# thesteve0/llm-fine-tune-distributed

Measured on AMD Instinct MI355X. Metric: samples/sec SmolLM3-3B full SFT bf16 (DDP), higher is better.
Workload: dtype bf16

## Files before the change

csrc/attention.hip:

```cpp
#include "common.h"

#include <cstring>

namespace sftamd {

namespace attn {

constexpr int D = 128;
constexpr int ROWB = D * 2;
constexpr float LOG2E = 1.4426950408889634f;
constexpr float LN2 = 0.6931471805599453f;

__device__ __forceinline__ int swz(int row, int ch) {
  return ch ^ (((row & 3) << 2) | ((0x78 >> (2 * ((row >> 2) & 3))) & 3));
}
__device__ __forceinline__ int img_off(int row, int ch) { return row * ROWB + 16 * swz(row, ch); }

__device__ __forceinline__ f32x4 mfma(const bf16x8& a, const bf16x8& b, const f32x4& c) {
  return __builtin_amdgcn_mfma_f32_16x16x32_bf16(a, b, c, 0, 0, 0);
}

template <int R, int NT>
__device__ __forceinline__ void stage(char* lds, const u16* __restrict__ g, long ld, int nvalid, int tid) {
#pragma unroll
  for (int it = 0; it < (R * 16) / NT; ++it) {
    const int idx = tid + it * NT;
    const int r = idx >> 4, ch = idx & 15;
    uint4 v = make_uint4(0, 0, 0, 0);
    if (r < nvalid) v = *(const uint4*)(g + (long)r * ld + ch * 8);
    *(uint4*)(lds + img_off(r, ch)) = v;
  }
}


__device__ __forceinline__ bf16x8 pack_acc(const f32x4& t0, const f32x4& t1) {
  typedef __attribute__((ext_vector_type(4))) unsigned w4;
  return __builtin_bit_cast(bf16x8, w4{pk2bf(t0[0], t0[1]), pk2bf(t0[2], t0[3]), pk2bf(t1[0], t1[1]), pk2bf(t1[2], t1[3])});
}

__device__ __forceinline__ bf16x8 load_frag_global(const u16* p, bool ok) {
  if (!ok) return bf16x8{};
  return __builtin_bit_cast(bf16x8, *(const uint4*)p);
}

__device__ __forceinline__ void store4(u16* p, const f32x4& v, float s) {
  uint2 w;
  w.x = pk2bf(v[0] * s, v[1] * s);
  w.y = pk2bf(v[2] * s, v[3] * s);
  *(uint2*)p = w;
}


__global__ __launch_bounds__(256) void delta_kernel(const u16* __restrict__ dout, const u16* __restrict__ out,
                                                    float* __restrict__ delta, int total, int nq) {
  const long rowid = blockIdx.x * 16L + (threadIdx.x >> 4);
  const int sub = threadIdx.x & 15;
  float s = 0.f;
  const bool ok = rowid < (long)total * nq;
  if (ok) {
    const long base = rowid * D + sub * 8;
    float a[8], c[8];
    unpack8(*(const uint4*)(dout + base), a);
    unpack8(*(const uint4*)(out + base), c);
#pragma unroll
    for (int i = 0; i < 8; ++i) s += a[i] * c[i];
  }
#pragma unroll
  for (int o = 8; o > 0; o >>= 1) s += __shfl_xor(s, o, 16);
  if (ok && sub == 0) {
    const long m = rowid / nq;
    const int h = (int)(rowid - m * nq);
    delta[(long)h * total + m] = s;
  }
}

constexpr float THR = 8.f;

struct Offs {
  int row[4];
  int tr[8];
  __device__ __forceinline__ void init(int lane) {
    const int g = lane >> 4, r = lane & 15;
#pragma unroll
    for (int s = 0; s < 4; ++s) row[s] = img_off(r, 4 * s + g);
    const int q = r >> 2, p = r & 3, r0 = 4 * g + q;
#pragma unroll
    for (int dt = 0; dt < 8; ++dt) tr[dt] = img_off(r0, 2 * dt + (p >> 1)) + 8 * (p & 1);
  }
};

__device__ __forceinline__ bf16x8 lds_row(const char* base, int off) { return *(const bf16x8*)(base + off); }

__device__ __forceinline__ bf16x8 lds_tr(const char* base, int off) {
  typedef __attribute__((address_space(3))) s16x4 lds_s4;
  s16x4 lo = __builtin_amdgcn_ds_read_tr16_b64_v4i16((lds_s4*)(base + off));
  s16x4 hi = __builtin_amdgcn_ds_read_tr16_b64_v4i16((lds_s4*)(base + off + 16 * ROWB));
  typedef __attribute__((ext_vector_type(8))) short s16x8;
  s16x8 v = {lo[0], lo[1], lo[2], lo[3], hi[0], hi[1], hi[2], hi[3]};
  return __builtin_bit_cast(bf16x8, v);
}

__device__ __forceinline__ void vm_drain() { __builtin_amdgcn_s_waitcnt(0x0F70); }

typedef float f32x2 __attribute__((ext_vector_type(2)));
__device__ __forceinline__ float max3f(float a, float b, float c) {
  float r;
  asm("v_max3_f32 %0, %1, %2, %3" : "=v"(r) : "v"(a), "v"(b), "v"(c));
  return r;
}

template <int R, int NT>
struct Stage {
  static constexpr int N = (R * 16) / NT;
  uint4 v[N];
  __device__ __forceinline__ void load(const u16* __restrict__ g, long ld, int nvalid, int tid) {
    const int r = tid >> 4, ch = tid & 15;
    const u16* p = g + (long)r * ld + ch * 8;
    if (nvalid >= R) {
#pragma unroll
      for (int it = 0; it < N; ++it) v[it] = *(const uint4*)(p + (long)it * (NT / 16) * ld);
    } else {
#pragma unroll
      for (int it = 0; it < N; ++it)
        v[it] = (r + it * (NT / 16) < nvalid) ? *(const uint4*)(p + (long)it * (NT / 16) * ld) : make_uint4(0, 0, 0, 0);
    }
  }
  __device__ __forceinline__ void store(char* lds, int tid) const {
    const int off = img_off(tid >> 4, tid & 15);
#pragma unroll
    for (int it = 0; it < N; ++it) *(uint4*)(lds + off + it * (NT / 16) * ROWB) = v[it];
  }
};


typedef __amdgpu_buffer_rsrc_t rsrc_t;
__device__ __forceinline__ rsrc_t make_rsrc(const void* p, long bytes) {
  const unsigned long long a = (unsigned long long)p;
  const unsigned lo = __builtin_amdgcn_readfirstlane((unsigned)a), hi = __builtin_amdgcn_readfirstlane((unsigned)(a >> 32));
  const unsigned n = __builtin_amdgcn_readfirstlane((unsigned)(bytes < 0 ? 0 : bytes));
  return __builtin_amdgcn_make_buffer_rsrc((void*)(((unsigned long long)hi << 32) | lo), 0, n, 0x00020000);
}
__device__ __forceinline__ void bdma16(rsrc_t r, char* dst, unsigned voff, unsigned soff) {
  __builtin_amdgcn_raw_ptr_buffer_load_lds(r, (__attribute__((address_space(3))) void*)dst, 16, voff, soff, 0, 0);
}
__device__ __forceinline__ bf16x8 bload16(rsrc_t r, unsigned voff) {
  const auto v = __builtin_amdgcn_raw_buffer_load_b128(r, voff, 0, 0);
  return __builtin_bit_cast(bf16x8, v);
}

typedef __attribute__((ext_vector_type(16))) float f32x16;

__device__ __forceinline__ f32x16 mfma32(const bf16x8& a, const bf16x8& b, const f32x16& c) {
  return __builtin_amdgcn_mfma_f32_32x32x16_bf16(a, b, c, 0, 0, 0);
}

struct Offs32 {
  int k[8];
  int v[8];
  __device__ __forceinline__ void init(int lane) {
    const int c = lane & 31, hi = lane >> 5, a = lane >> 4, q = (lane & 15) >> 2, p = lane & 3;
#pragma unroll
    for (int s = 0; s < 8; ++s) k[s] = img_off(c, 2 * s + hi);
#pragma unroll
    for (int db = 0; db < 4; ++db)
#pragma unroll
      for (int part = 0; part < 2; ++part)
        v[2 * db + part] = img_off(8 * part + 4 * hi + q, 4 * db + 2 * (a & 1) + (p >> 1)) + 8 * (p & 1);
  }
};

__device__ __forceinline__ bf16x8 lds_tr2(const char* base, int lo, int hi) {
  typedef __attribute__((address_space(3))) s16x4 lds_s4;
  s16x4 a = __builtin_amdgcn_ds_read_tr16_b64_v4i16((lds_s4*)(base + lo));
  s16x4 b = __builtin_amdgcn_ds_read_tr16_b64_v4i16((lds_s4*)(base + hi));
  typedef __attribute__((ext_vector_type(8))) short s16x8;
  s16x8 v = {a[0], a[1], a[2], a[3], b[0], b[1], b[2], b[3]};
  return __builtin_bit_cast(bf16x8, v);
}

typedef __attribute__((ext_vector_type(4))) unsigned u32x4;
__device__ __forceinline__ u32x4 pack8w(const f32x16& t, int base) {
  return u32x4{pk2bf(t[base], t[base + 1]), pk2bf(t[base + 2], t[base + 3]), pk2bf(t[base + 4], t[base + 5]),
               pk2bf(t[base + 6], t[base + 7])};
}
__device__ __forceinline__ bf16x8 pack8(const f32x16& t, int base) {
  return __builtin_bit_cast(bf16x8, pack8w(t, base));
}

__device__ __forceinline__ float swap32max(float x) {
  auto a = __builtin_amdgcn_permlane32_swap(__float_as_uint(x), __float_as_uint(x), false, false);
  return fmaxf(__uint_as_float(a[0]), __uint_as_float(a[1]));
}
__device__ __forceinline__ float swap32sum(float x) {
  auto a = __builtin_amdgcn_permlane32_swap(__float_as_uint(x), __float_as_uint(x), false, false);
  return __uint_as_float(a[0]) + __uint_as_float(a[1]);
}

__device__ __forceinline__ void store_t21(u16* row, const f32x16 (&a)[4], float s, bool ok) {
  const int hi = (threadIdx.x >> 5) & 1;
#pragma unroll
  for (int db = 0; db < 4; ++db)
#pragma unroll
    for (int u = 0; u < 2; ++u) {
      const int i0 = 8 * u;
      const unsigned ax = pk2bf(a[db][i0] * s, a[db][i0 + 1] * s);
      const unsigned ay = pk2bf(a[db][i0 + 2] * s, a[db][i0 + 3] * s);
      const unsigned bx = pk2bf(a[db][i0 + 4] * s, a[db][i0 + 5] * s);
      const unsigned by = pk2bf(a[db][i0 + 6] * s, a[db][i0 + 7] * s);
      const auto rx = __builtin_amdgcn_permlane32_swap(ax, bx, false, false);
      const auto ry = __builtin_amdgcn_permlane32_swap(ay, by, false, false);
      if (ok) *(uint4*)(row + 32 * db + 16 * u + 8 * hi) = make_uint4(rx[0], ry[0], rx[1], ry[1]);
    }
}

__device__ __forceinline__ void fwd32_step(const char* __restrict__ cur, char* __restrict__ nxt, bool pre, rsrc_t kv,
                                           unsigned voffk, unsigned voffv, unsigned rowb, int wave, int k0, int lastkey,
                                           bool need_mask, int rel, float sl2, const Offs32& off,
                                           const bf16x8 (&qf)[8], f32x16 (&o)[4], float& m, float& l) {
  constexpr int TB = 64 * ROWB;
  if (pre) {
#pragma unroll
    for (int j = 0; j < 4; ++j) {
      const unsigned so = (unsigned)(k0 + 64 + 16 * j) * rowb;
      bdma16(kv, nxt + (wave + 4 * j) * 1024, voffk, so);
      bdma16(kv, nxt + TB + (wave + 4 * j) * 1024, voffv, so);
    }
  }
  if (k0 > lastkey) return;
  const bool two = k0 + 32 <= lastkey;
  const char* Ks = cur;
  const char* Vs = cur + TB;
  f32x16 s[2];
  s[0] = mfma32(lds_row(Ks, off.k[0]), qf[0], f32x16{});
#pragma unroll
  for (int st = 1; st < 8; ++st) s[0] = mfma32(lds_row(Ks, off.k[st]), qf[st], s[0]);
  if (two) {
    s[1] = mfma32(lds_row(Ks, off.k[0] + 32 * ROWB), qf[0], f32x16{});
#pragma unroll
    for (int st = 1; st < 8; ++st) s[1] = mfma32(lds_row(Ks, off.k[st] + 32 * ROWB), qf[st], s[1]);
  } else {
#pragma unroll
    for (int i = 0; i < 16; ++i) s[1][i] = -INFINITY;
  }
  if (need_mask) {
#pragma unroll
    for (int kb = 0; kb < 2; ++kb)
#pragma unroll
      for (int i = 0; i < 16; ++i)
        s[kb][i] = 32 * kb + (i & 3) + 8 * (i >> 2) > rel ? -INFINITY : s[kb][i];
  }
  float mx = max3f(s[0][0], s[0][1], s[0][2]);
#pragma unroll
  for (int i = 3; i < 15; i += 2) mx = max3f(mx, s[0][i], s[0][i + 1]);
  mx = max3f(mx, s[0][15], s[1][0]);
#pragma unroll
  for (int i = 1; i < 15; i += 2) mx = max3f(mx, s[1][i], s[1][i + 1]);
  mx = fmaxf(mx, s[1][15]);
  const float tmax = swap32max(mx) * sl2;
  if (__any(tmax > m + THR)) {
    const float mnew = fmaxf(m, tmax);
    const float alpha = exp2f(m - mnew);
    l *= alpha;
#pragma unroll
    for (int db = 0; db < 4; ++db) o[db] *= alpha;
    m = mnew;
  }
  float acc0 = 0.f, acc1 = 0.f;
#pragma unroll
  for (int kb = 0; kb < 2; ++kb)
#pragma unroll
    for (int i = 0; i < 16; i += 2) {
      const float p0 = exp2f(__builtin_fmaf(s[kb][i], sl2, -m));
      const float p1 = exp2f(__builtin_fmaf(s[kb][i + 1], sl2, -m));
      s[kb][i] = p0;
      s[kb][i + 1] = p1;
      acc0 += p0;
      acc1 += p1;
    }
  l += acc0 + acc1;
#pragma unroll
  for (int ks = 0; ks < 4; ++ks) {
    if (ks >= 2 && !two) break;
    const bf16x8 pb = pack8(s[ks >> 1], 8 * (ks & 1));
#pragma unroll
    for (int db = 0; db < 4; ++db)
      o[db] = mfma32(lds_tr2(Vs, off.v[2 * db] + 16 * ks * ROWB, off.v[2 * db + 1] + 16 * ks * ROWB), pb, o[db]);
  }
}

template <int HW>
__global__ __launch_bounds__(256, 2) void fwd32_kernel(const u16* __restrict__ qkv, u16* __restrict__ out,
                                                       float* __restrict__ lse, const int* __restrict__ cu, int nq,
                                                       int nkv, int total, float sl2, int causal) {
  constexpr int PB = 4 / HW, TB = 64 * ROWB;
  __shared__ __attribute__((aligned(16))) char smem[4 * TB];
  const int b = blockIdx.y, qb = gridDim.z - 1 - blockIdx.z;
  const int start = cu[b], len = cu[b + 1] - start;
  SFT_DASSERT(start >= 0 && len >= 0 && start + len <= total);
  const int q0 = qb * 32 * PB;
  if (q0 >= len) return;
  const int tid = threadIdx.x, lane = tid & 63, wave = __builtin_amdgcn_readfirstlane(tid >> 6), hi = lane >> 5;
  const int h = blockIdx.x * HW + wave % HW;
  const int kvh = (blockIdx.x * HW) / (nq / nkv);
  const long ld = (long)(nq + 2 * nkv) * D;
  const int wq0 = q0 + 32 * (wave / HW);
  const int qi = wq0 + (lane & 31);
  const bool qok = qi < len;
  const int nkb = (len + 63) / 64;
  const int nkt = causal ? min((min(q0 + 32 * PB, len) - 1) / 64 + 1, nkb) : nkb;
  const int lastkey = causal ? min(wq0 + 31, len - 1) : len - 1;
  const int lim = causal ? min(len - 1, qi) : len - 1;
  Offs32 off;
  off.init(lane);
  const unsigned rowb = (unsigned)ld * 2;
  bf16x8 qf[8];
  {
    const rsrc_t qr = make_rsrc(qkv + (long)start * ld + h * D, (long)(len - 1) * ld * 2 + ROWB);
    const unsigned vo = (unsigned)qi * rowb + 16 * hi;
#pragma unroll
    for (int st = 0; st < 8; ++st) qf[st] = bload16(qr, vo + 32 * st);
  }
  const rsrc_t kv = make_rsrc(qkv + (long)start * ld + (nq + kvh) * D, (long)len * ld * 2 - (long)(nq + kvh) * ROWB);
  const int r0 = 4 * wave + (lane >> 4);
  const unsigned voffk = (unsigned)r0 * rowb + 16 * swz(r0, lane & 15), voffv = voffk + nkv * ROWB;
#pragma unroll
  for (int j = 0; j < 4; ++j) {
    bdma16(kv, smem + (wave + 4 * j) * 1024, voffk, 16 * j * rowb);
    bdma16(kv, smem + TB + (wave + 4 * j) * 1024, voffv, 16 * j * rowb);
  }
  vm_drain();
  f32x16 o[4];
#pragma unroll
  for (int db = 0; db < 4; ++db)
#pragma unroll
    for (int i = 0; i < 16; ++i) o[db][i] = 0.f;
  float m = -1e30f, l = 0.f;
  __syncthreads();
  for (int kt = 0; kt < nkt; ++kt) {
    const int k0 = kt * 64;
    const bool pre = kt + 1 < nkt;
    const bool need_mask = (k0 + 64 > len) || (causal && k0 + 63 > wq0);
    fwd32_step(smem + (kt & 1) * 2 * TB, smem + ((kt + 1) & 1) * 2 * TB, pre, kv, voffk, voffv, rowb, wave, k0,
               lastkey, need_mask, lim - k0 - 4 * hi, sl2, off, qf, o, m, l);
    if (pre) vm_drain();
    __syncthreads();
  }
  l = swap32sum(l);
  const float inv = 1.f / l;
  store_t21(out + (long)(start + qi) * nq * D + h * D, o, inv, qok);
  if (qok && hi == 0) lse[(long)h * total + start + qi] = (m + log2f(l)) * LN2;
}

template <int NW>
__global__ __launch_bounds__(NW * 64) void bwd_dq3_kernel(const u16* __restrict__ qkv, const u16* __restrict__ dout,
                                                          const float* __restrict__ lse,
                                                          const float* __restrict__ delta, const int* __restrict__ cu,
                                                          u16* __restrict__ dqkv, int nq, int nkv, int total,
                                                          float sl2, float scale, int causal) {
  constexpr int NT = NW * 64, BM = NW * 16, TB = 64 * ROWB;
  __shared__ __attribute__((aligned(16))) char smem[2 * TB];
  char* Ks = smem;
  char* Vs = smem + TB;
  const int h = blockIdx.x, b = blockIdx.y, qb = gridDim.z - 1 - blockIdx.z;
  const int start = cu[b], len = cu[b + 1] - start;
  SFT_DASSERT(start >= 0 && len >= 0 && start + len <= total);
  const int q0 = qb * BM;
  if (q0 >= len) return;
  const int kvh = h / (nq / nkv);
  const long ld = (long)(nq + 2 * nkv) * D;
  const long ldo = (long)nq * D;
  const int tid = threadIdx.x, lane = tid & 63, wave = tid >> 6, g = lane >> 4;
  const int wfirst = q0 + wave * 16;
  const int qrow = wfirst + (lane & 15);
  const bool qok = qrow < len;
  const u16* kbase = qkv + (long)start * ld + (nq + kvh) * D;
  const u16* vbase = qkv + (long)start * ld + (nq + nkv + kvh) * D;
  const int nkb = (len + 63) / 64;
  const int nkt = causal ? min((q0 + BM + 63) / 64, nkb) : nkb;
  Offs off;
  off.init(lane);
  {
    Stage<64, NT> tk, tv;
    tk.load(kbase, ld, len, tid);
    tv.load(vbase, ld, len, tid);
    tk.store(Ks, tid);
    tv.store(Vs, tid);
  }
  bf16x8 qf[4], df[4];
  {
    const u16* qp = qkv + (long)(start + qrow) * ld + h * D + 8 * g;
    const u16* dp = dout + (long)(start + qrow) * ldo + h * D + 8 * g;
#pragma unroll
    for (int s = 0; s < 4; ++s) {
      qf[s] = load_frag_global(qp + 32 * s, qok);
      df[s] = load_frag_global(dp + 32 * s, qok);
    }
  }
  const float lse2 = qok ? lse[(long)h * total + start + qrow] * LOG2E : 0.f;
  const float dl = qok ? delta[(long)h * total + start + qrow] : 0.f;
  f32x4 dq[8];
#pragma unroll
  for (int dt = 0; dt < 8; ++dt) dq[dt] = f32x4{0.f, 0.f, 0.f, 0.f};
  __syncthreads();
  for (int kt = 0; kt < nkt; ++kt) {
    const int k0 = kt * 64;
    const bool pre = kt + 1 < nkt;
    Stage<64, NT> tk, tv;
    if (pre) {
      tk.load(kbase + (long)(k0 + 64) * ld, ld, len - k0 - 64, tid);
      tv.load(vbase + (long)(k0 + 64) * ld, ld, len - k0 - 64, tid);
    }
    if (!causal || k0 <= wfirst + 15) {
      f32x4 sc[4], dp[4];
#pragma unroll
      for (int nt = 0; nt < 4; ++nt) {
        sc[nt] = f32x4{0.f, 0.f, 0.f, 0.f};
        dp[nt] = f32x4{0.f, 0.f, 0.f, 0.f};
#pragma unroll
        for (int s = 0; s < 4; ++s) {
          sc[nt] = mfma(lds_row(Ks, off.row[s] + nt * 16 * ROWB), qf[s], sc[nt]);
          dp[nt] = mfma(lds_row(Vs, off.row[s] + nt * 16 * ROWB), df[s], dp[nt]);
        }
      }
      const bool need_mask = (k0 + 64 > len) || (causal && k0 + 63 > wfirst) || (q0 + BM > len);
#pragma unroll
      for (int nt = 0; nt < 4; ++nt)
#pragma unroll
        for (int i = 0; i < 4; ++i) {
          float p = exp2f(fmaf(sc[nt][i], sl2, -lse2));
          if (need_mask) {
            const int key = k0 + 16 * nt + 4 * g + i;
            if (key >= len || (causal && key > qrow) || !qok) p = 0.f;
          }
          dp[nt][i] = p * (dp[nt][i] - dl);
        }
#pragma unroll
      for (int ks = 0; ks < 2; ++ks) {
        const bf16x8 db = pack_acc(dp[2 * ks], dp[2 * ks + 1]);
#pragma unroll
        for (int dt = 0; dt < 8; ++dt) dq[dt] = mfma(lds_tr(Ks, off.tr[dt] + ks * 32 * ROWB), db, dq[dt]);
      }
    }
    if (pre) {
      __syncthreads();
      tk.store(Ks, tid);
      tv.store(Vs, tid);
    }
    __syncthreads();
  }
  if (qok) {
    u16* qp = dqkv + (long)(start + qrow) * ld + h * D + 4 * g;
#pragma unroll
    for (int dt = 0; dt < 8; ++dt) store4(qp + 16 * dt, dq[dt], scale);
  }
}

__device__ __forceinline__ void rope_bwd32(f32x16 (&a)[4], const float* cs, const float* sn, float s) {
  const int hi = (threadIdx.x >> 5) & 1;
#pragma unroll
  for (int d4 = 0; d4 < 2; ++d4)
#pragma unroll
    for (int m = 0; m < 4; ++m) {
      const int d = 32 * d4 + 8 * m + 4 * hi;
      const float4 c4 = *(const float4*)(cs + d), s4 = *(const float4*)(sn + d);
      const float c[4] = {c4.x, c4.y, c4.z, c4.w}, n[4] = {s4.x, s4.y, s4.z, s4.w};
#pragma unroll
      for (int t = 0; t < 4; ++t) {
        const int i = 4 * m + t;
        const float x = a[d4][i] * s, y = a[d4 + 2][i] * s;
        a[d4][i] = x * c[t] + y * n[t];
        a[d4 + 2][i] = y * c[t] - x * n[t];
      }
    }
}

__device__ __forceinline__ void dq32_step(const char* __restrict__ cur, char* __restrict__ nxt, bool pre, bool active,
                                          rsrc_t kr, rsrc_t sr, unsigned voffk, unsigned voffs, unsigned rowb,
                                          unsigned rows, int k0n, int wave, const Offs32& off, int sofs,
                                          f32x16 (&dq)[4]) {
  constexpr int TB = 64 * ROWB, SB = 64 * 64;
  if (pre) {
#pragma unroll
    for (int j = 0; j < 4; ++j) {
      bdma16(kr, nxt + (wave + 4 * j) * 1024, voffk, (unsigned)(k0n + 16 * j) * rowb);
      bdma16(sr, nxt + TB + wave * SB + j * 1024, voffs, (unsigned)(k0n + 16 * j) * rows);
    }
  }
  if (!active) return;
  const char* Ks = cur;
  const char* Ss = cur + TB + wave * SB;
#pragma unroll
  for (int ks = 0; ks < 4; ++ks) {
    const bf16x8 sb = lds_tr2(Ss, sofs + ks * 16 * 64, sofs + ks * 16 * 64 + 8 * 64);
#pragma unroll
    for (int d4 = 0; d4 < 4; ++d4)
      dq[d4] = mfma32(lds_tr2(Ks, off.v[2 * d4] + ks * 16 * ROWB, off.v[2 * d4 + 1] + ks * 16 * ROWB), sb, dq[d4]);
  }
}

template <int HW>
__global__ __launch_bounds__(256, 2) void bwd_dq32_kernel(const u16* __restrict__ qkv, const u16* __restrict__ dst,
                                                          const int* __restrict__ cu, u16* __restrict__ dqkv, int nq,
                                                          int nkv, int lp, float scale, int causal,
                                                          const float* __restrict__ rcos,
                                                          const float* __restrict__ rsin) {
  constexpr int PB = 4 / HW, TB = 64 * ROWB, SB = 64 * 64, STG = TB + 4 * SB;
  __shared__ __attribute__((aligned(16))) char smem[2 * STG];
  const int b = blockIdx.y, qb = gridDim.z - 1 - blockIdx.z;
  const int start = cu[b], len = cu[b + 1] - start;
  const int q0 = qb * 32 * PB;
  if (q0 >= len) return;
  const int tid = threadIdx.x, lane = tid & 63, wave = __builtin_amdgcn_readfirstlane(tid >> 6), hi = lane >> 5;
  const int h = blockIdx.x * HW + wave % HW;
  const int kvh = (blockIdx.x * HW) / (nq / nkv);
  const long ld = (long)(nq + 2 * nkv) * D;
  const int wq0 = q0 + 32 * (wave / HW);
  const int qi = wq0 + (lane & 31);
  SFT_DASSERT(wq0 + 32 <= lp);
  const int lastq = min(wq0 + 31, len - 1);
  const u16* kbase = qkv + (long)start * ld + (nq + kvh) * D;
  const u16* sbase = dst + (long)(b * nq + h) * lp * lp + wq0;
  const int nkb = (len + 63) / 64;
  const int nkt = causal ? min((min(q0 + 32 * PB, len) - 1) / 64 + 1, nkb) : nkb;
  Offs32 off;
  off.init(lane);
  const int sofs = (4 * hi + ((lane & 15) >> 2)) * 64 + 32 * ((lane >> 4) & 1) + 8 * (lane & 3);
  const int r0 = 4 * wave + (lane >> 4);
  const unsigned rowb = (unsigned)ld * 2, rows = (unsigned)lp * 2;
  const rsrc_t kr = make_rsrc(kbase, (long)(len - 1) * ld * 2 + ROWB);
  const rsrc_t sr = make_rsrc(sbase, (long)(len - 1) * lp * 2 + 64);
  const unsigned voffk = (unsigned)r0 * rowb + 16 * swz(r0, lane & 15);
  const unsigned voffs = (unsigned)(lane >> 2) * rows + 16 * (lane & 3);
  f32x16 dq[4];
#pragma unroll
  for (int d4 = 0; d4 < 4; ++d4)
#pragma unroll
    for (int i = 0; i < 16; ++i) dq[d4][i] = 0.f;
  dq32_step(smem + STG, smem, true, false, kr, sr, voffk, voffs, rowb, rows, 0, wave, off, sofs, dq);
  vm_drain();
  __syncthreads();
  for (int kt = 0; kt < nkt; ++kt) {
    const int k0 = kt * 64;
    const bool pre = kt + 1 < nkt;
    dq32_step(smem + (kt & 1) * STG, smem + ((kt + 1) & 1) * STG, pre, !causal || k0 <= lastq, kr, sr, voffk, voffs,
              rowb, rows, k0 + 64, wave, off, sofs, dq);
    if (pre) vm_drain();
    __syncthreads();
  }
  const bool qok = qi < len;
  float s = scale;
  if (rcos != nullptr && qok) {
    const long tr = (long)(start + qi) * (D / 2);
    rope_bwd32(dq, rcos + tr, rsin + tr, scale);
    s = 1.f;
  }
  store_t21(dqkv + (long)(start + qi) * ld + h * D, dq, s, qok);
}

__device__ __forceinline__ void dkdv32_step(const char* __restrict__ cur, char* __restrict__ nxt, bool pre,
                                            rsrc_t qr, rsrc_t orr, unsigned vq0, unsigned vq1, unsigned vo0,
                                            unsigned vo1, unsigned qso, unsigned oso, unsigned rowb, unsigned rowo,
                                            int wv, const float* lsrc, const float* dsrc, int gl, int q0, int len,
                                            int causal, int kw0, int key, float sl2, u16* drow,
                                            const Offs32& off, const bf16x8 (&kf)[8], const char* Vk,
                                            f32x16 (&dk)[4], f32x16 (&dv)[4]) {
  constexpr int TB = 64 * ROWB;
  float pl = 0.f, pd = 0.f;
  if (pre) {
#pragma unroll
    for (int j = 0; j < 8; ++j) {
      bdma16(qr, nxt + (wv + 2 * j) * 1024, (j & 1) ? vq1 : vq0, qso + 16 * (j >> 1) * rowb);
      bdma16(orr, nxt + TB + (wv + 2 * j) * 1024, (j & 1) ? vo1 : vo0, oso + 16 * (j >> 1) * rowo);
    }
    if (gl < 64 && lsrc != nullptr) {
      pl = lsrc[gl];
      pd = dsrc[gl];
    }
  }
  const char* Qs = cur;
  const char* Os = cur + TB;
  const float* Ls = (const float*)(cur + 2 * TB);
  const float* Dl = Ls + 64;
  const int hi = (threadIdx.x >> 5) & 1;
  const bool wds = __builtin_amdgcn_readfirstlane((int)(drow != nullptr));
#pragma unroll 1
  for (int qb = 0; qb < 2; ++qb) {
    f32x16 s, dp;
#pragma unroll
    for (int i = 0; i < 16; ++i) s[i] = dp[i] = 0.f;
#pragma unroll
    for (int st = 0; st < 8; ++st) {
      s = mfma32(lds_row(Qs, off.k[st] + qb * 32 * ROWB), kf[st], s);
      dp = mfma32(lds_row(Os, off.k[st] + qb * 32 * ROWB), lds_row(Vk, off.k[st]), dp);
    }
    const int qbase = q0 + 32 * qb + 4 * hi;
    const int lo = (causal ? key : 0) - qbase, hq = len - 1 - qbase;
    const bool need_mask = (q0 + 32 * qb + 31 >= len) || (causal && kw0 + 31 > q0 + 32 * qb);
#pragma unroll
    for (int m = 0; m < 4; ++m) {
      const float4 L4 = *(const float4*)(Ls + 32 * qb + 8 * m + 4 * hi);
      const float4 D4 = *(const float4*)(Dl + 32 * qb + 8 * m + 4 * hi);
      const float L[4] = {L4.x, L4.y, L4.z, L4.w}, Dd[4] = {D4.x, D4.y, D4.z, D4.w};
#pragma unroll
      for (int t = 0; t < 4; ++t) {
        const int i = 4 * m + t;
        const float p = exp2f(__builtin_fmaf(s[i], sl2, -L[t]));
        dp[i] = p * (dp[i] - Dd[t]);
        s[i] = p;
      }
    }
    if (need_mask) {
      int vlo = lo, vhi = hq;
      asm volatile("" : "+v"(vlo), "+v"(vhi));
#pragma unroll
      for (int i = 0; i < 16; ++i) {
        const int o = 8 * (i >> 2) + (i & 3);
        if (o < vlo || o > vhi) s[i] = dp[i] = 0.f;
      }
    }
#pragma unroll
    for (int sub = 0; sub < 2; ++sub) {
      const u32x4 dw = pack8w(dp, 8 * sub);
      if (wds) {
        const auto rx = __builtin_amdgcn_permlane32_swap(dw[0], dw[2], false, false);
        const auto ry = __builtin_amdgcn_permlane32_swap(dw[1], dw[3], false, false);
        *(uint4*)(drow + 32 * qb + 16 * sub + 8 * hi) = make_uint4(rx[0], ry[0], rx[1], ry[1]);
      }
      const bf16x8 pb = pack8(s, 8 * sub), db = __builtin_bit_cast(bf16x8, dw);
      const int ko = (2 * qb + sub) * 16 * ROWB;
#pragma unroll
      for (int d4 = 0; d4 < 4; ++d4) {
        dv[d4] = mfma32(lds_tr2(Os, off.v[2 * d4] + ko, off.v[2 * d4 + 1] + ko), pb, dv[d4]);
        dk[d4] = mfma32(lds_tr2(Qs, off.v[2 * d4] + ko, off.v[2 * d4 + 1] + ko), db, dk[d4]);
      }
    }
  }
  if (pre && gl < 64) {
    float* Ln = (float*)(nxt + 2 * TB);
    asm volatile("" : "+v"(pl));
    Ln[gl] = pl * LOG2E;
    Ln[64 + gl] = pd;
  }
}

template <int G>
__global__ __launch_bounds__(128 * G, 1) void bwd_dkdv32_kernel(
    const u16* __restrict__ qkv, const u16* __restrict__ dout, const float* __restrict__ lse,
    const float* __restrict__ delta, const int* __restrict__ cu, u16* __restrict__ dqkv, int nq, int nkv, int total,
    float sl2, float scale, int causal, u16* __restrict__ dst, int lp, const float* __restrict__ rcos,
    const float* __restrict__ rsin) {
  constexpr int TB = 64 * ROWB, GB = 2 * TB + 2 * 64 * 4;
  __shared__ __attribute__((aligned(16))) char smem[G * 2 * GB + TB];
  const int tid = threadIdx.x, lane = tid & 63, w = __builtin_amdgcn_readfirstlane(tid >> 6), grp = w >> 1, kh = w & 1;
  const int gl = tid & 127;
  const int hi = lane >> 5;
  char* base = smem + grp * 2 * GB;
  const int kvh = blockIdx.x, b = blockIdx.y, kb = blockIdx.z;
  const int start = cu[b], len = cu[b + 1] - start;
  SFT_DASSERT(start >= 0 && len >= 0 && start + len <= total);
  const int k0 = kb * 64;
  if (k0 >= len) return;
  const int rep = nq / nkv, hpg = rep / G;
  const long ld = (long)(nq + 2 * nkv) * D;
  const long ldo = (long)nq * D;
  const int kw0 = k0 + 32 * kh, key = kw0 + (lane & 31);
  const bool kok = key < len;
  const int qt0 = causal ? kb : 0, nqt = (len + 63) / 64, nt = nqt - qt0, niter = hpg * nt;
  Offs32 off;
  off.init(lane);
  int h = kvh * rep + grp * hpg, qt = qt0;
  const int qr0 = 4 * kh + (lane >> 4);
  const unsigned rowb = (unsigned)ld * 2, rowo = (unsigned)ldo * 2;
  const rsrc_t qr = make_rsrc(qkv + (long)start * ld, (long)(len - 1) * ld * 2 + (long)nq * ROWB);
  const rsrc_t orr = make_rsrc(dout + (long)start * ldo, (long)len * ldo * 2);
  const unsigned sw0 = 16 * swz(qr0, lane & 15), sw1 = 16 * swz(qr0 + 8, lane & 15);
  const unsigned vq0 = (unsigned)qr0 * rowb + sw0, vq1 = (unsigned)(qr0 + 8) * rowb + sw1;
  const unsigned vo0 = (unsigned)qr0 * rowo + sw0, vo1 = (unsigned)(qr0 + 8) * rowo + sw1;
  {
    const int q0 = qt0 * 64, qv = len - q0;
#pragma unroll
    for (int j = 0; j < 8; ++j) {
      bdma16(qr, base + (kh + 2 * j) * 1024, (j & 1) ? vq1 : vq0, (unsigned)(q0 + 16 * (j >> 1)) * rowb + h * ROWB);
      bdma16(orr, base + TB + (kh + 2 * j) * 1024, (j & 1) ? vo1 : vo0, (unsigned)(q0 + 16 * (j >> 1)) * rowo + h * ROWB);
    }
    if (gl < 64) {
      float* Ls = (float*)(base + 2 * TB);
      Ls[gl] = gl < qv ? lse[(long)h * total + start + q0 + gl] * LOG2E : 0.f;
      Ls[64 + gl] = gl < qv ? delta[(long)h * total + start + q0 + gl] : 0.f;
    }
  }
  bf16x8 kf[8];
  char* Vk = smem + G * 2 * GB + kh * 32 * ROWB;
  {
    const rsrc_t kr = make_rsrc(qkv + (long)start * ld + (nq + kvh) * D, (long)(len - 1) * ld * 2 + (long)(nkv + 1) * ROWB);
    const unsigned vo = (unsigned)key * rowb + 16 * hi;
#pragma unroll
    for (int st = 0; st < 8; ++st) kf[st] = bload16(kr, vo + 32 * st);
    const int vr = 4 * w + (lane >> 4);
    const unsigned vv0 = (unsigned)(k0 + vr) * rowb + nkv * ROWB + 16 * swz(vr, lane & 15);
    const unsigned vv1 = (unsigned)(k0 + vr) * rowb + nkv * ROWB + 16 * swz(vr + 8, lane & 15);
#pragma unroll
    for (int j = 0; j < 8 / G; ++j)
      bdma16(kr, smem + G * 2 * GB + (w + 2 * G * j) * 1024, (G == 1 && (j & 1)) ? vv1 : vv0,
             (unsigned)(8 * G * j) * rowb);
  }
  vm_drain();
  f32x16 dk[4], dv[4];
#pragma unroll
  for (int d4 = 0; d4 < 4; ++d4)
#pragma unroll
    for (int i = 0; i < 16; ++i) dk[d4][i] = dv[d4][i] = 0.f;
  __syncthreads();
  for (int it = 0; it < niter; ++it) {
    const int q0 = qt * 64;
    const bool pre = it + 1 < niter;
    int hn = h, qtn = qt + 1;
    if (qtn == nqt) {
      qtn = qt0;
      ++hn;
    }
    const int qn = qtn * 64;
    const long lo = (long)hn * total + start + qn;
    const bool lok = pre && qn + gl < len;
    u16* drow = dst != nullptr ? dst + ((long)(b * nq + h) * lp + key) * lp + q0 : nullptr;
    dkdv32_step(base + (it & 1) * GB, base + ((it + 1) & 1) * GB, pre, qr, orr, vq0, vq1, vo0, vo1,
                (unsigned)qn * rowb + hn * ROWB, (unsigned)qn * rowo + hn * ROWB, rowb, rowo, kh,
                lok ? lse + lo : nullptr, delta + lo, gl, q0, len, causal, kw0, key, sl2, drow, off, kf, Vk, dk,
                dv);
    if (pre) vm_drain();
    __syncthreads();
    h = hn;
    qt = qtn;
  }
  if constexpr (G == 2) {
    float4* xk = (float4*)smem;
    float4* xv = xk + 2 * 16 * 64;
    if (grp == 1) {
#pragma unroll
      for (int d4 = 0; d4 < 4; ++d4)
#pragma unroll
        for (int v = 0; v < 4; ++v) {
          const int ix = (kh * 16 + 4 * d4 + v) * 64 + lane;
          xk[ix] = make_float4(dk[d4][4 * v], dk[d4][4 * v + 1], dk[d4][4 * v + 2], dk[d4][4 * v + 3]);
          xv[ix] = make_float4(dv[d4][4 * v], dv[d4][4 * v + 1], dv[d4][4 * v + 2], dv[d4][4 * v + 3]);
        }
    }
    __syncthreads();
    if (grp == 1) return;
#pragma unroll
    for (int d4 = 0; d4 < 4; ++d4)
#pragma unroll
      for (int v = 0; v < 4; ++v) {
        const int ix = (kh * 16 + 4 * d4 + v) * 64 + lane;
        const float4 a = xk[ix], c = xv[ix];
        dk[d4][4 * v] += a.x;
        dk[d4][4 * v + 1] += a.y;
        dk[d4][4 * v + 2] += a.z;
        dk[d4][4 * v + 3] += a.w;
        dv[d4][4 * v] += c.x;
        dv[d4][4 * v + 1] += c.y;
        dv[d4][4 * v + 2] += c.z;
        dv[d4][4 * v + 3] += c.w;
      }
  }
  float ks = scale;
  if (rcos != nullptr && kok) {
    const long tr = (long)(start + key) * (D / 2);
    rope_bwd32(dk, rcos + tr, rsin + tr, scale);
    ks = 1.f;
  }
  store_t21(dqkv + (long)(start + key) * ld + (nq + kvh) * D, dk, ks, kok);
  store_t21(dqkv + (long)(start + key) * ld + (nq + nkv + kvh) * D, dv, 1.f, kok);
}

static void launch_dkdv(const u16* qkv, const u16* dout, const float* lse, const float* delta, const int* cu,
                        u16* dqkv, int nq, int nkv, int total, int nseq, int max_seqlen, float sl2, float scale,
                        int causal, u16* dst, int lp, hipStream_t st, const float* rcos = nullptr,
                        const float* rsin = nullptr) {
  dim3 grid(nkv, nseq, (max_seqlen + 63) / 64);
  if ((nq / nkv) % 2 == 0)
    bwd_dkdv32_kernel<2><<<grid, 256, 0, st>>>(qkv, dout, lse, delta, cu, dqkv, nq, nkv, total, sl2, scale, causal,
                                               dst, lp, rcos, rsin);
  else
    bwd_dkdv32_kernel<1><<<grid, 128, 0, st>>>(qkv, dout, lse, delta, cu, dqkv, nq, nkv, total, sl2, scale, causal,
                                               dst, lp, rcos, rsin);
}

}

static void check_attn_args(const at::Tensor& qkv, const at::Tensor& cu, int64_t nq, int64_t nkv, int64_t hd) {
  SFT_CHECK_CUDA(qkv);
  SFT_CHECK_BF16(qkv);
  SFT_CHECK_CONTIG(qkv);
  SFT_CHECK(hd == attn::D, "flash attention kernel is built for head_dim 128, got ", hd);
  SFT_CHECK(nq % nkv == 0, "nq must be a multiple of nkv");
  SFT_CHECK(qkv.dim() == 2 && qkv.size(1) == (nq + 2 * nkv) * hd, "qkv must be [M, (nq+2nkv)*hd]");
  SFT_CHECK(cu.scalar_type() == at::kInt && cu.is_cuda() && cu.dim() == 1 && cu.numel() >= 2, "cu_seqlens int32");
}

static long attn_ds_budget() {
  const char* e = std::getenv("SFTAMD_ATTN_DS_MB");
  return (e && e[0] ? atol(e) : 2048L) * 1024L * 1024L;
}

std::tuple<at::Tensor, at::Tensor> flash_fwd(const at::Tensor& qkv, const at::Tensor& cu, int64_t max_seqlen,
                                             int64_t nq, int64_t nkv, int64_t hd, double scale, bool causal) {
  check_attn_args(qkv, cu, nq, nkv, hd);
  const int total = qkv.size(0);
  const int nseq = cu.numel() - 1;
  auto out = at::empty({total, nq * hd}, qkv.options());
  auto lse = at::empty({nq, total}, qkv.options().dtype(at::kFloat));
  if (total == 0 || max_seqlen == 0) return {out, lse};
  const float sl2 = (float)scale * attn::LOG2E;
  auto cu_c = cu.contiguous();
  const u16* q = (const u16*)qkv.data_ptr();
  u16* o = (u16*)out.data_ptr();
  float* lp = lse.data_ptr<float>();
  const int* cp = cu_c.data_ptr<int>();
  const int ca = causal ? 1 : 0;
  SFT_TRACE("attn.fwd32");
  const int rep = nq / nkv, hw = rep % 4 == 0 ? 4 : rep % 2 == 0 ? 2 : 1, span = 32 * (4 / hw);
  dim3 g(nq / hw, nseq, (max_seqlen + span - 1) / span);
  if (hw == 4) attn::fwd32_kernel<4><<<g, 256, 0, cur_stream()>>>(q, o, lp, cp, nq, nkv, total, sl2, ca);
  else if (hw == 2) attn::fwd32_kernel<2><<<g, 256, 0, cur_stream()>>>(q, o, lp, cp, nq, nkv, total, sl2, ca);
  else attn::fwd32_kernel<1><<<g, 256, 0, cur_stream()>>>(q, o, lp, cp, nq, nkv, total, sl2, ca);
  SFT_LAUNCH_CHECK();
  return {out, lse};
}

static at::Tensor flash_bwd_impl(const at::Tensor& dout, const at::Tensor& qkv, const at::Tensor& out,
                                 const at::Tensor& lse, const at::Tensor& cu, int64_t max_seqlen, int64_t nq,
                                 int64_t nkv, int64_t hd, double scale, bool causal, const float* rcos,
                                 const float* rsin, bool& rope_done, const c10::optional<at::Tensor>& delta_in) {
  rope_done = false;
  check_attn_args(qkv, cu, nq, nkv, hd);
  SFT_CHECK_CONTIG(dout);
  SFT_CHECK_CONTIG(out);
  SFT_CHECK(dout.sizes() == out.sizes() && out.size(1) == nq * hd, "dout/out shape");
  const int total = qkv.size(0);
  const int nseq = cu.numel() - 1;
  auto dqkv = at::empty_like(qkv);
  if (total == 0 || max_seqlen == 0) return dqkv;
  at::Tensor delta;
  if (delta_in.has_value() && delta_in->defined()) {
    delta = *delta_in;
    SFT_CHECK(delta.scalar_type() == at::kFloat && delta.is_contiguous() && delta.dim() == 2 && delta.size(0) == nq &&
                  delta.size(1) == total && delta.device() == qkv.device(),
              "flash_bwd: delta must be contiguous fp32 [n_q, total]");
  } else {
    SFT_TRACE("attn.delta_kernel");
    delta = at::empty({nq, total}, qkv.options().dtype(at::kFloat));
    const long rows = (long)total * nq;
    attn::delta_kernel<<<(rows + 15) / 16, 256, 0, cur_stream()>>>((const u16*)dout.data_ptr(),
                                                                    (const u16*)out.data_ptr(), delta.data_ptr<float>(),
                                                                    total, nq);
    SFT_LAUNCH_CHECK();
  }
  const float sl2 = (float)scale * attn::LOG2E;
  auto cu_c = cu.contiguous();
  const u16* q = (const u16*)qkv.data_ptr();
  const u16* dO = (const u16*)dout.data_ptr();
  const long lp = (max_seqlen + 127) / 128 * 128;
  const long ds_bytes = (long)nseq * nq * lp * lp * 2;
  if (ds_bytes <= attn_ds_budget()) {
    auto dst = at::empty({ds_bytes / 2}, qkv.options());
    const bool rope = rcos != nullptr;
    SFT_TRACE("attn.dkdv32");
    SFT_TRACE("attn.dq32");
    if (rope) SFT_TRACE("attn.bwd_rope_epi");
    attn::launch_dkdv(q, dO, lse.data_ptr<float>(), delta.data_ptr<float>(), cu_c.data_ptr<int>(),
                       (u16*)dqkv.data_ptr(), nq, nkv, total, nseq, max_seqlen, sl2, (float)scale, causal ? 1 : 0,
                       (u16*)dst.data_ptr(), (int)lp, cur_stream(), rcos, rsin);
    SFT_LAUNCH_CHECK();
    {
      const int rep = nq / nkv, hw = rep % 4 == 0 ? 4 : rep % 2 == 0 ? 2 : 1, span = 32 * (4 / hw);
      dim3 g(nq / hw, nseq, (max_seqlen + span - 1) / span);
      const u16* ds = (const u16*)dst.data_ptr();
      u16* dx = (u16*)dqkv.data_ptr();
      const int* cp = cu_c.data_ptr<int>();
      const int ca = causal ? 1 : 0;
      if (hw == 4) attn::bwd_dq32_kernel<4><<<g, 256, 0, cur_stream()>>>(q, ds, cp, dx, nq, nkv, (int)lp, (float)scale, ca, rcos, rsin);
      else if (hw == 2) attn::bwd_dq32_kernel<2><<<g, 256, 0, cur_stream()>>>(q, ds, cp, dx, nq, nkv, (int)lp, (float)scale, ca, rcos, rsin);
      else attn::bwd_dq32_kernel<1><<<g, 256, 0, cur_stream()>>>(q, ds, cp, dx, nq, nkv, (int)lp, (float)scale, ca, rcos, rsin);
    }
    SFT_LAUNCH_CHECK();
    rope_done = rope;
    return dqkv;
  }
  SFT_TRACE("attn.dq3");
  dim3 gq3(nq, nseq, (max_seqlen + 127) / 128);
  attn::bwd_dq3_kernel<8><<<gq3, 512, 0, cur_stream()>>>(q, dO, lse.data_ptr<float>(), delta.data_ptr<float>(),
                                                         cu_c.data_ptr<int>(), (u16*)dqkv.data_ptr(), nq, nkv, total,
                                                         sl2, (float)scale, causal ? 1 : 0);
  SFT_LAUNCH_CHECK();
  attn::launch_dkdv(q, dO, lse.data_ptr<float>(), delta.data_ptr<float>(), cu_c.data_ptr<int>(),
                     (u16*)dqkv.data_ptr(), nq, nkv, total, nseq, max_seqlen, sl2, (float)scale, causal ? 1 : 0,
                     nullptr, 0, cur_stream());
  SFT_LAUNCH_CHECK();
  return dqkv;
}

at::Tensor flash_bwd(const at::Tensor& dout, const at::Tensor& qkv, const at::Tensor& out, const at::Tensor& lse,
                     const at::Tensor& cu, int64_t max_seqlen, int64_t nq, int64_t nkv, int64_t hd, double scale,
                     bool causal, const c10::optional<at::Tensor>& delta) {
  bool rope_done;
  return flash_bwd_impl(dout, qkv, out, lse, cu, max_seqlen, nq, nkv, hd, scale, causal, nullptr, nullptr, rope_done,
                        delta);
}

void rope_(at::Tensor qkv, const at::Tensor& cos, const at::Tensor& sin, int64_t n_q, int64_t n_kv, int64_t head_dim,
           bool inverse);

at::Tensor flash_bwd_rope(const at::Tensor& dout, const at::Tensor& qkv, const at::Tensor& out, const at::Tensor& lse,
                          const at::Tensor& cu, int64_t max_seqlen, int64_t nq, int64_t nkv, int64_t hd, double scale,
                          bool causal, const at::Tensor& cos, const at::Tensor& sin,
                          const c10::optional<at::Tensor>& delta) {
  SFT_CHECK(cos.scalar_type() == at::kFloat && sin.scalar_type() == at::kFloat && cos.is_contiguous() &&
                sin.is_contiguous() && cos.is_cuda() && sin.is_cuda(),
            "flash_bwd_rope: contiguous fp32 cos / sin");
  SFT_CHECK(cos.numel() == qkv.size(0) * hd / 2 && sin.numel() == cos.numel(), "flash_bwd_rope: cos / sin [total, hd/2]");
  bool rope_done;
  auto dqkv = flash_bwd_impl(dout, qkv, out, lse, cu, max_seqlen, nq, nkv, hd, scale, causal, cos.data_ptr<float>(),
                             sin.data_ptr<float>(), rope_done, delta);
  if (!rope_done) rope_(dqkv, cos, sin, nq, nkv, hd, true);
  return dqkv;
}

TORCH_LIBRARY_IMPL(sftamd, CUDA, m) {
  m.impl("flash_fwd", &flash_fwd);
  m.impl("flash_bwd", &flash_bwd);
  m.impl("flash_bwd_rope", &flash_bwd_rope);
}

}
```

Baseline: 118.4.

## Split dK/dV backward query halves across extra waves with LDS reduction

Adds a 512-thread dK/dV backward kernel that gives each 32-row half of the 64-query tile to its own wave, where before one wave looped over both halves. Partial dK/dV accumulators are then reduced through shared memory in two rounds. The DMA prefetch of the next Q/dO tile is interleaved with the QK/dOV MFMA steps through a per-step callback. The aim is more waves in flight to hide latency, at the cost of more threads per block, extra LDS reduction traffic and barriers. The old two-group kernel stays available behind an environment variable.

```diff
diff --git a/csrc/attention.hip b/csrc/attention.hip
--- a/csrc/attention.hip
+++ b/csrc/attention.hip
@@ -557,6 +557,68 @@
   store_t21(dqkv + (long)(start + qi) * ld + h * D, dq, s, qok);
 }
 
+struct NoPiece {
+  __device__ __forceinline__ void operator()(int) const {}
+};
+template <class Piece>
+__device__ __forceinline__ void dkdv32_half(const char* __restrict__ Qs, const char* __restrict__ Os,
+                                            const float* __restrict__ Ls, const float* __restrict__ Dl, int qh0,
+                                            int len, int causal, int kw0, int key, float sl2, u16* drow, bool wds,
+                                            const Offs32& off, const bf16x8 (&kf)[8], const char* Vk,
+                                            f32x16 (&dk)[4], f32x16 (&dv)[4], const Piece& piece) {
+  const int hi = (threadIdx.x >> 5) & 1;
+  f32x16 s, dp;
+#pragma unroll
+  for (int i = 0; i < 16; ++i) s[i] = dp[i] = 0.f;
+#pragma unroll
+  for (int st = 0; st < 8; ++st) {
+    piece(st);
+    s = mfma32(lds_row(Qs, off.k[st]), kf[st], s);
+    dp = mfma32(lds_row(Os, off.k[st]), lds_row(Vk, off.k[st]), dp);
+  }
+  const int qbase = qh0 + 4 * hi;
+  const int lo = (causal ? key : 0) - qbase, hq = len - 1 - qbase;
+  const bool need_mask = (qh0 + 31 >= len) || (causal && kw0 + 31 > qh0);
+#pragma unroll
+  for (int m = 0; m < 4; ++m) {
+    const float4 L4 = *(const float4*)(Ls + 8 * m + 4 * hi);
+    const float4 D4 = *(const float4*)(Dl + 8 * m + 4 * hi);
+    const float L[4] = {L4.x, L4.y, L4.z, L4.w}, Dd[4] = {D4.x, D4.y, D4.z, D4.w};
+#pragma unroll
+    for (int t = 0; t < 4; ++t) {
+      const int i = 4 * m + t;
+      const float p = exp2f(__builtin_fmaf(s[i], sl2, -L[t]));
+      dp[i] = p * (dp[i] - Dd[t]);
+      s[i] = p;
+    }
+  }
+  if (need_mask) {
+    int vlo = lo, vhi = hq;
+    asm volatile("" : "+v"(vlo), "+v"(vhi));
+#pragma unroll
+    for (int i = 0; i < 16; ++i) {
+      const int o = 8 * (i >> 2) + (i & 3);
+      if (o < vlo || o > vhi) s[i] = dp[i] = 0.f;
+    }
+  }
+#pragma unroll
+  for (int sub = 0; sub < 2; ++sub) {
+    const u32x4 dw = pack8w(dp, 8 * sub);
+    if (wds) {
+      const auto rx = __builtin_amdgcn_permlane32_swap(dw[0], dw[2], false, false);
+      const auto ry = __builtin_amdgcn_permlane32_swap(dw[1], dw[3], false, false);
+      *(uint4*)(drow + 16 * sub + 8 * hi) = make_uint4(rx[0], ry[0], rx[1], ry[1]);
+    }
+    const bf16x8 pb = pack8(s, 8 * sub), db = __builtin_bit_cast(bf16x8, dw);
+    const int ko = sub * 16 * ROWB;
+#pragma unroll
+    for (int d4 = 0; d4 < 4; ++d4) {
+      dv[d4] = mfma32(lds_tr2(Os, off.v[2 * d4] + ko, off.v[2 * d4 + 1] + ko), pb, dv[d4]);
+      dk[d4] = mfma32(lds_tr2(Qs, off.v[2 * d4] + ko, off.v[2 * d4 + 1] + ko), db, dk[d4]);
+    }
+  }
+}
+
 __device__ __forceinline__ void dkdv32_step(const char* __restrict__ cur, char* __restrict__ nxt, bool pre,
                                             rsrc_t qr, rsrc_t orr, unsigned vq0, unsigned vq1, unsigned vo0,
                                             unsigned vo1, unsigned qso, unsigned oso, unsigned rowb, unsigned rowo,
@@ -581,60 +643,11 @@
   const char* Os = cur + TB;
   const float* Ls = (const float*)(cur + 2 * TB);
   const float* Dl = Ls + 64;
-  const int hi = (threadIdx.x >> 5) & 1;
   const bool wds = __builtin_amdgcn_readfirstlane((int)(drow != nullptr));
 #pragma unroll 1
-  for (int qb = 0; qb < 2; ++qb) {
-    f32x16 s, dp;
-#pragma unroll
-    for (int i = 0; i < 16; ++i) s[i] = dp[i] = 0.f;
-#pragma unroll
-    for (int st = 0; st < 8; ++st) {
-      s = mfma32(lds_row(Qs, off.k[st] + qb * 32 * ROWB), kf[st], s);
-      dp = mfma32(lds_row(Os, off.k[st] + qb * 32 * ROWB), lds_row(Vk, off.k[st]), dp);
-    }
-    const int qbase = q0 + 32 * qb + 4 * hi;
-    const int lo = (causal ? key : 0) - qbase, hq = len - 1 - qbase;
-    const bool need_mask = (q0 + 32 * qb + 31 >= len) || (causal && kw0 + 31 > q0 + 32 * qb);
-#pragma unroll
-    for (int m = 0; m < 4; ++m) {
-      const float4 L4 = *(const float4*)(Ls + 32 * qb + 8 * m + 4 * hi);
-      const float4 D4 = *(const float4*)(Dl + 32 * qb + 8 * m + 4 * hi);
-      const float L[4] = {L4.x, L4.y, L4.z, L4.w}, Dd[4] = {D4.x, D4.y, D4.z, D4.w};
-#pragma unroll
-      for (int t = 0; t < 4; ++t) {
-        const int i = 4 * m + t;
-        const float p = exp2f(__builtin_fmaf(s[i], sl2, -L[t]));
-        dp[i] = p * (dp[i] - Dd[t]);
-        s[i] = p;
-      }
-    }
-    if (need_mask) {
-      int vlo = lo, vhi = hq;
-      asm volatile("" : "+v"(vlo), "+v"(vhi));
-#pragma unroll
-      for (int i = 0; i < 16; ++i) {
-        const int o = 8 * (i >> 2) + (i & 3);
-        if (o < vlo || o > vhi) s[i] = dp[i] = 0.f;
-      }
-    }
-#pragma unroll
-    for (int sub = 0; sub < 2; ++sub) {
-      const u32x4 dw = pack8w(dp, 8 * sub);
-      if (wds) {
-        const auto rx = __builtin_amdgcn_permlane32_swap(dw[0], dw[2], false, false);
-        const auto ry = __builtin_amdgcn_permlane32_swap(dw[1], dw[3], false, false);
-        *(uint4*)(drow + 32 * qb + 16 * sub + 8 * hi) = make_uint4(rx[0], ry[0], rx[1], ry[1]);
-      }
-      const bf16x8 pb = pack8(s, 8 * sub), db = __builtin_bit_cast(bf16x8, dw);
-      const int ko = (2 * qb + sub) * 16 * ROWB;
-#pragma unroll
-      for (int d4 = 0; d4 < 4; ++d4) {
-        dv[d4] = mfma32(lds_tr2(Os, off.v[2 * d4] + ko, off.v[2 * d4 + 1] + ko), pb, dv[d4]);
-        dk[d4] = mfma32(lds_tr2(Qs, off.v[2 * d4] + ko, off.v[2 * d4 + 1] + ko), db, dk[d4]);
-      }
-    }
-  }
+  for (int qb = 0; qb < 2; ++qb)
+    dkdv32_half(Qs + qb * 32 * ROWB, Os + qb * 32 * ROWB, Ls + 32 * qb, Dl + 32 * qb, q0 + 32 * qb, len, causal, kw0,
+                key, sl2, drow + 32 * qb, wds, off, kf, Vk, dk, dv, NoPiece{});
   if (pre && gl < 64) {
     float* Ln = (float*)(nxt + 2 * TB);
     asm volatile("" : "+v"(pl));
@@ -773,17 +786,192 @@
   store_t21(dqkv + (long)(start + key) * ld + (nq + nkv + kvh) * D, dv, 1.f, kok);
 }
 
+__device__ __forceinline__ void dkdv32w_step(const char* __restrict__ cur, char* __restrict__ nxt, bool pre,
+                                             rsrc_t qr, rsrc_t orr, unsigned vq, unsigned vo, unsigned qso,
+                                             unsigned oso, unsigned rowb, unsigned rowo, int wv, int qb,
+                                             const float* xsrc, float xmul, int lane, int q0, int len, int causal,
+                                             int kw0, int key, float sl2, u16* drow, const Offs32& off,
+                                             const bf16x8 (&kf)[8], const char* Vk, f32x16 (&dk)[4],
+                                             f32x16 (&dv)[4]) {
+  constexpr int TB = 64 * ROWB;
+  float px = 0.f;
+  if (pre && xsrc != nullptr) px = xsrc[lane];
+  const bool wds = __builtin_amdgcn_readfirstlane((int)(drow != nullptr));
+  const char* Qs = cur + qb * 32 * ROWB;
+  const float* Ls = (const float*)(cur + 2 * TB) + 32 * qb;
+  dkdv32_half(Qs, Qs + TB, Ls, Ls + 64, q0 + 32 * qb, len, causal, kw0, key, sl2, drow + 32 * qb, wds, off, kf, Vk, dk,
+              dv, [&](int st) {
+                const int j = st >> 1;
+                if (st & 1) bdma16(orr, nxt + TB + (wv + 4 * j) * 1024, vo, oso + 16 * j * rowo);
+                else bdma16(qr, nxt + (wv + 4 * j) * 1024, vq, qso + 16 * j * rowb);
+              });
+  if (pre && wv < 2) {
+    float* Ln = (float*)(nxt + 2 * TB);
+    asm volatile("" : "+v"(px));
+    Ln[64 * wv + lane] = px * xmul;
+  }
+}
+
+__global__ __launch_bounds__(512, 1) void bwd_dkdv32w_kernel(
+    const u16* __restrict__ qkv, const u16* __restrict__ dout, const float* __restrict__ lse,
+    const float* __restrict__ delta, const int* __restrict__ cu, u16* __restrict__ dqkv, int nq, int nkv, int total,
+    float sl2, float scale, int causal, u16* __restrict__ dst, int lp, const float* __restrict__ rcos,
+    const float* __restrict__ rsin) {
+  constexpr int TB = 64 * ROWB, GB = 2 * TB + 2 * 64 * 4;
+  __shared__ __attribute__((aligned(16))) char smem[4 * GB + TB];
+  static_assert(4 * 2 * 16 * 64 * 16 <= 4 * GB, "four waves' dK / dV partials must fit in the stages");
+  const int tid = threadIdx.x, lane = tid & 63, w = __builtin_amdgcn_readfirstlane(tid >> 6);
+  const int kh = w & 1, grp = (w >> 1) & 1, qb = w >> 2, wv = kh + 2 * qb;
+  const int hi = lane >> 5;
+  char* base = smem + grp * 2 * GB;
+  const int kvh = blockIdx.x, b = blockIdx.y, kb = blockIdx.z;
+  const int start = cu[b], len = cu[b + 1] - start;
+  SFT_DASSERT(start >= 0 && len >= 0 && start + len <= total);
+  const int k0 = kb * 64;
+  if (k0 >= len) return;
+  const int rep = nq / nkv, hpg = rep / 2;
+  const long ld = (long)(nq + 2 * nkv) * D;
+  const long ldo = (long)nq * D;
+  const int kw0 = k0 + 32 * kh, key = kw0 + (lane & 31);
+  const bool kok = key < len;
+  const int qt0 = causal ? kb : 0, nqt = (len + 63) / 64, nt = nqt - qt0, niter = hpg * nt;
+  Offs32 off;
+  off.init(lane);
+  int h = kvh * rep + grp * hpg, qt = qt0;
+  const int qr0 = 4 * wv + (lane >> 4);
+  const unsigned rowb = (unsigned)ld * 2, rowo = (unsigned)ldo * 2;
+  const rsrc_t qr = make_rsrc(qkv + (long)start * ld, (long)(len - 1) * ld * 2 + (long)nq * ROWB);
+  const rsrc_t orr = make_rsrc(dout + (long)start * ldo, (long)len * ldo * 2);
+  const unsigned sw = 16 * swz(qr0, lane & 15);
+  const unsigned vq = (unsigned)qr0 * rowb + sw, vo = (unsigned)qr0 * rowo + sw;
+  const float* xbase = wv == 0 ? lse : delta;
+  const float xmul = wv == 0 ? LOG2E : 1.f;
+  {
+    const int q0 = qt0 * 64, qv = len - q0;
+#pragma unroll
+    for (int j = 0; j < 4; ++j) {
+      bdma16(qr, base + (wv + 4 * j) * 1024, vq, (unsigned)(q0 + 16 * j) * rowb + h * ROWB);
+      bdma16(orr, base + TB + (wv + 4 * j) * 1024, vo, (unsigned)(q0 + 16 * j) * rowo + h * ROWB);
+    }
+    if (wv < 2) {
+      float* Ls = (float*)(base + 2 * TB);
+      Ls[64 * wv + lane] = lane < qv ? xbase[(long)h * total + start + q0 + lane] * xmul : 0.f;
+    }
+  }
+  bf16x8 kf[8];
+  const char* Vk = smem + 4 * GB + kh * 32 * ROWB;
+  {
+    const rsrc_t kr = make_rsrc(qkv + (long)start * ld + (nq + kvh) * D, (long)(len - 1) * ld * 2 + (long)(nkv + 1) * ROWB);
+    const unsigned ko = (unsigned)key * rowb + 16 * hi;
+#pragma unroll
+    for (int st = 0; st < 8; ++st) kf[st] = bload16(kr, ko + 32 * st);
+    const int vr = 4 * w + (lane >> 4);
+    const unsigned vv = (unsigned)(k0 + vr) * rowb + nkv * ROWB + 16 * swz(vr, lane & 15);
+#pragma unroll
+    for (int j = 0; j < 2; ++j) bdma16(kr, smem + 4 * GB + (w + 8 * j) * 1024, vv, (unsigned)(32 * j) * rowb);
+  }
+  vm_drain();
+  f32x16 dk[4], dv[4];
+#pragma unroll
+  for (int d4 = 0; d4 < 4; ++d4)
+#pragma unroll
+    for (int i = 0; i < 16; ++i) dk[d4][i] = dv[d4][i] = 0.f;
+  __syncthreads();
+  for (int it = 0; it < niter; ++it) {
+    const int q0 = qt * 64;
+    const bool pre = it + 1 < niter;
+    int hn = h, qtn = qt + 1;
+    if (qtn == nqt) {
+      qtn = qt0;
+      ++hn;
+    }
+    if (!pre) {
+      hn = h;
+      qtn = qt;
+    }
+    const int qn = qtn * 64;
+    const bool xok = pre && wv < 2 && qn + lane < len;
+    u16* drow = dst != nullptr ? dst + ((long)(b * nq + h) * lp + key) * lp + q0 : nullptr;
+    dkdv32w_step(base + (it & 1) * GB, base + ((it + 1) & 1) * GB, pre, qr, orr, vq, vo,
+                 (unsigned)qn * rowb + hn * ROWB, (unsigned)qn * rowo + hn * ROWB, rowb, rowo, wv, qb,
+                 xok ? xbase + (long)hn * total + start + qn : nullptr, xmul, lane, q0, len, causal, kw0, key, sl2,
+                 drow, off, kf, Vk, dk, dv);
+    vm_drain();
+    __syncthreads();
+    h = hn;
+    qt = qtn;
+  }
+  float4* xch = (float4*)smem;
+#pragma unroll
+  for (int rnd = 0; rnd < 2; ++rnd) {
+    const bool give = rnd == 0 ? qb == 1 : (qb == 0 && grp == 1);
+    const bool take = rnd == 0 ? qb == 0 : (qb == 0 && grp == 0);
+    float4* xk = xch + (rnd == 0 ? kh + 2 * grp : kh) * (2 * 16 * 64);
+    float4* xv = xk + 16 * 64;
+    if (give) {
+#pragma unroll
+      for (int d4 = 0; d4 < 4; ++d4)
+#pragma unroll
+        for (int v = 0; v < 4; ++v) {
+          const int ix = (4 * d4 + v) * 64 + lane;
+          xk[ix] = make_float4(dk[d4][4 * v], dk[d4][4 * v + 1], dk[d4][4 * v + 2], dk[d4][4 * v + 3]);
+          xv[ix] = make_float4(dv[d4][4 * v], dv[d4][4 * v + 1], dv[d4][4 * v + 2], dv[d4][4 * v + 3]);
+        }
+    }
+    __syncthreads();
+    if (take) {
+#pragma unroll
+      for (int d4 = 0; d4 < 4; ++d4)
+#pragma unroll
+        for (int v = 0; v < 4; ++v) {
+          const int ix = (4 * d4 + v) * 64 + lane;
+          const float4 a = xk[ix], c = xv[ix];
+          dk[d4][4 * v] += a.x;
+          dk[d4][4 * v + 1] += a.y;
+          dk[d4][4 * v + 2] += a.z;
+          dk[d4][4 * v + 3] += a.w;
+          dv[d4][4 * v] += c.x;
+          dv[d4][4 * v + 1] += c.y;
+          dv[d4][4 * v + 2] += c.z;
+          dv[d4][4 * v + 3] += c.w;
+        }
+    }
+    if (rnd == 0) __syncthreads();
+  }
+  if (w >= 2) return;
+  float ks = scale;
+  if (rcos != nullptr && kok) {
+    const long tr = (long)(start + key) * (D / 2);
+    rope_bwd32(dk, rcos + tr, rsin + tr, scale);
+    ks = 1.f;
+  }
+  store_t21(dqkv + (long)(start + key) * ld + (nq + kvh) * D, dk, ks, kok);
+  store_t21(dqkv + (long)(start + key) * ld + (nq + nkv + kvh) * D, dv, 1.f, kok);
+}
+
+static bool attn_dkdv_one_wave() {
+  const char* e = std::getenv("SFTAMD_ATTN_DKDV_1W");
+  return e && e[0] && e[0] != '0';
+}
+
 static void launch_dkdv(const u16* qkv, const u16* dout, const float* lse, const float* delta, const int* cu,
                         u16* dqkv, int nq, int nkv, int total, int nseq, int max_seqlen, float sl2, float scale,
                         int causal, u16* dst, int lp, hipStream_t st, const float* rcos = nullptr,
                         const float* rsin = nullptr) {
   dim3 grid(nkv, nseq, (max_seqlen + 63) / 64);
-  if ((nq / nkv) % 2 == 0)
+  if ((nq / nkv) % 2 != 0) {
+    SFT_TRACE("attn.dkdv32.g1");
+    bwd_dkdv32_kernel<1><<<grid, 128, 0, st>>>(qkv, dout, lse, delta, cu, dqkv, nq, nkv, total, sl2, scale, causal,
+                                               dst, lp, rcos, rsin);
+  } else if (attn_dkdv_one_wave()) {
+    SFT_TRACE("attn.dkdv32.g2");
     bwd_dkdv32_kernel<2><<<grid, 256, 0, st>>>(qkv, dout, lse, delta, cu, dqkv, nq, nkv, total, sl2, scale, causal,
                                                dst, lp, rcos, rsin);
-  else
-    bwd_dkdv32_kernel<1><<<grid, 128, 0, st>>>(qkv, dout, lse, delta, cu, dqkv, nq, nkv, total, sl2, scale, causal,
-                                               dst, lp, rcos, rsin);
+  } else {
+    SFT_TRACE("attn.dkdv32.2w");
+    bwd_dkdv32w_kernel<<<grid, 512, 0, st>>>(qkv, dout, lse, delta, cu, dqkv, nq, nkv, total, sl2, scale, causal, dst,
+                                             lp, rcos, rsin);
+  }
 }
 
 }
```

After: 118.7, median of 6. About the same (+0.2%).
